# Z-T-WANG/DeepReinforcementLearningControlOfQuantumCartpoles

Hardware: AMD Instinct MI355X
Metric: env-steps/sec (whole node), inverted-harmonic grid=512 batch=65536; 1/2/4/8 GPU (higher is better)
Workload: dtype f64; 1 GPU; inverted_harmonic N=512 per-GPU batch=65536 dt=1/1440 80 physics steps + moments per step (metric); global_batch=65536, seq_len=512, parallelism=env-shard1, world_size_seen=1

## Files before the change

deepreinforcementlearningcontrolofquantumcartpoles_amd/csrc/qcart_api.cpp:

```cpp
#include <hip/hip_runtime.h>

#include <algorithm>
#include <cmath>
#include <cstdlib>
#include <cstring>
#include <mutex>
#include <string>
#include <vector>

#include "../../include/qcart.h"
#include "qcart_kargs.hpp"
#include "qcart_tables.hpp"

using namespace qcart;

namespace {
constexpr int kMaxSlots = 64;
constexpr int kShortCallSteps = 10;
constexpr int64_t kShortCallBatch = 4096;
constexpr int64_t kSpreadBatch = 1024;
std::mutex g_err_mu;
std::string g_create_err;

void set_create_err(const std::string& s) {
// ... 156 lines not shown
    if ((rc = upload(h, &h->d_kb, kb.data(), kb.size()))) return rc;
    return QC_OK;
}

int build_all_actions(qc_handle* h) {
    std::vector<double> forces;
    for (auto& a : h->acts) forces.push_back(a.force);
    if (forces.empty())
        for (int a = 0; a < h->p.n_actions; a++)
            forces.push_back((double)(a - h->p.n_actions / 2) * (h->p.f_max / (double)(h->p.n_actions / 2)));
    h->acts.assign(forces.size(), ActHost());
    for (size_t i = 0; i < forces.size(); i++) {
        int rc = build_action(h->op, h->p.dt, forces[i], h->mirror, h->acts[i], h->err);
        if (rc) return rc;
    }
    return QC_OK;
}

KArgs base_args(const qc_handle* h) {
    KArgs a;
    std::memset(&a, 0, sizeof(a));
    const qc_params& p = h->p;
    const OpHost& op = h->op;
    a.B = p.batch;
    a.env_offset = p.env_offset;
    a.seed = p.seed;
    a.ctr = h->d_ctr;
    a.N = op.N;
    a.Npad = op.Npad;
    a.n_slots = (int32_t)h->acts.size();
    a.mirror = h->mirror ? 1 : 0;
    a.bnd_len = op.fock ? kFockBnd : kGridBnd;
    a.win_lo = a.win_hi = 0;
    if (!op.fock && p.xth > 0) {
        const int c = op.N / 2, w = (int)std::nearbyint(p.xth / op.h);
        a.win_lo = c - w;
        a.win_hi = c + w;
    }
    a.moment_order = op.fock ? 0 : p.moment_order;
    {
        int lf = 0, lb = 0;
        for (auto& s : h->acts) {
            lf = std::max(lf, s.kf);
            lb = std::max(lb, s.kb);
        }
        const bool f32 = p.precision == QC_FP32;
        const uint32_t es = f32 ? 8u : 16u;
        const SlotLayout L = slot_layout(op.kl, op.Rs, op.family == QC_IHO, es, op.sym, op.lanes);
        const int NL = mode2_levels(op.kl);
        const size_t t1 = L.tf, t2 = L.tf + (size_t)(2 * NL + 2) * op.kl * op.kl * op.lanes * es;
        const size_t fx = op.fock ? (f32 ? 0 : (size_t)(op.R + 1 + (op.family == QC_IHO ? op.R : 0)) * kWave * 8)
                                  : (grid_rows_in_lds(op.R) ? (size_t)2 * op.R * kWave * 8 : 0);
        const size_t t4 = L.tf + (size_t)(NL + 1) * op.kl * op.kl * op.lanes * es;
        const size_t nzb = f32 ? 0 : (size_t)h->wpb * kNzLds, cap = 160 * 1024 - nzb;
        const bool m4 = !op.fock && !f32 && grid_rows_in_lds(op.R) && lf <= NL && t4 + fx <= cap;
        int mode = (t2 + fx <= cap && lf <= NL && lb <= NL) ? 2 : m4 ? 4 : (t1 + fx <= cap ? 1 : 0);
        if (const char* e = std::getenv("QCART_TAB_MODE")) {
            const int c = std::atoi(e);
            if (mode != 4 || c < 2) mode = std::min(mode, c);
        }
        a.tab_mode = mode;
        a.lds_fx = (uint32_t)(mode == 2 ? t2 : mode == 4 ? t4 : t1);
        a.lds_bytes = mode ? (uint32_t)(a.lds_fx + fx) : 0u;
        if (h->dual_img && mode >= 1) {
            a.lds_img = h->dual_img;
            a.lds_bytes = std::max(a.lds_bytes, 2u * h->dual_img);
        }
        a.lds_nz = 0;
        if (mode >= 1 && nzb) {
            a.lds_nz = (a.lds_bytes + 15u) & ~15u;
            a.lds_bytes = a.lds_nz + (uint32_t)nzb;
        }
    }
    a.precision = p.precision;
    a.order = nullptr;
    a.n_blocks = (uint32_t)((p.batch + h->wpb - 1) / h->wpb);
    a.n_obs = qc_n_obs(h);
    a.dt = p.dt;
    a.sqrt_dt = std::sqrt(p.dt);
    a.gamma = p.gamma;
    a.g4 = p.gamma / 4.;
    a.beta = std::sqrt(p.gamma / 2.);
    a.inv_sqrt2g = 1.0 / std::sqrt(2. * p.gamma);
    a.w = op.w;
    a.inv_sqrt_w = 1.0 / std::sqrt(op.w);
    a.c = op.c;
    a.h = op.fock ? 1.0 : op.h;
    const double dt = p.dt;
    a.x2h = op.family == QC_IHO ? -1.0 / op.c : 0.0;
    a.a2 = dt * dt * dt / 12.;
    a.a3 = dt * dt * dt * dt / 24.;
    a.a4 = dt * dt * dt * dt * dt / 80.;
    a.a5 = dt * dt * dt * dt * dt * dt / 360.;
    a.inv_sdt = 1.0 / a.sqrt_dt;
    a.inv_dt = 1.0 / dt;
    a.k_hisdt = 0.5 * a.inv_sdt;
    a.k_qisdt = 0.25 * a.inv_sdt;
    a.k_hidt = 0.5 * a.inv_dt;
    a.k_qidt = 0.25 * a.inv_dt;
    a.k_qdt = 0.25 * dt;
    a.k_qsdt = 0.25 * a.sqrt_dt;
    a.k_dz = a.sqrt_dt * dt * 0.5;
    a.k_sb = a.sqrt_dt * a.beta;
    a.b2 = a.a2 / a.a5;
    a.b3 = a.a3 / a.a5;
    a.b4 = a.a4 / a.a5;
    a.fail_thr = p.family == QC_HO ? 1e-3 : (p.family == QC_IHO ? 2e-3 : 5e-3);
// ... 699 lines not shown
```

deepreinforcementlearningcontrolofquantumcartpoles_amd/csrc/qcart_expt.hpp:

```cpp
#pragma once
#include <hip/hip_runtime.h>

#ifndef QCART_W8_MAX_R
#define QCART_W8_MAX_R 8
#endif
#ifndef QCART_W8_MAX_RG
#define QCART_W8_MAX_RG 9
#endif
#ifndef QCART_GRID_HC
#define QCART_GRID_HC 1
#endif
#ifndef QCART_GRID_KAR
#define QCART_GRID_KAR 0
#endif
#ifndef QCART_WKS_F32
#define QCART_WKS_F32 3
#endif
#ifndef QCART_SPLITM
#define QCART_SPLITM 1
#endif
#ifndef QCART_NZ_LDS
#define QCART_NZ_LDS 1
#endif
#ifndef QCART_MCONV_NT
#define QCART_MCONV_NT 2, 2, 1
#endif
#ifndef QCART_MCONV_NA
#define QCART_MCONV_NA 2, 1, 2
#endif
#ifndef QCART_MCONV_Q
#define QCART_MCONV_Q 4, 4, 4
#endif
#ifndef QCART_MFC_MT
#define QCART_MFC_MT 2
#endif
#ifndef QCART_MFC_NT
#define QCART_MFC_NT 2
#endif
#ifndef QCART_FC1_STAGE_K
#define QCART_FC1_STAGE_K 1
#endif

#ifdef QCART_STAMPS
namespace qcart {
__device__ unsigned long long qc_stamps[20];
}
#define QC_STAMP(ph)                                                                                 \
    do {                                                                                             \
        __builtin_amdgcn_sched_barrier(0);                                                           \
        unsigned long long t_;                                                                       \
        asm volatile("s_memtime %0\n\ts_waitcnt lgkmcnt(0)" : "=s"(t_)::"memory");                   \
        __builtin_amdgcn_sched_barrier(0);                                                           \
        st_acc[st_ph] += t_ - st_t;                                                                  \
        st_t = t_;                                                                                   \
        st_ph = (ph);                                                                                \
    } while (0)
#define QC_STAMP_BEGIN()                                                                             \
    unsigned long long st_acc[16] = {0}, st_t = 0;                                                   \
    int st_ph = 9;                                                                                   \
    asm volatile("s_memtime %0\n\ts_waitcnt lgkmcnt(0)" : "=s"(st_t)::"memory");                     \
    const unsigned long long st_loop0 = st_t
#define QC_KSTAMP_ENTRY()                                                                            \
    unsigned long long kst_t0;                                                                       \
    asm volatile("s_memtime %0\n\ts_waitcnt lgkmcnt(0)" : "=s"(kst_t0)::"memory")
#define QC_KSTAMP_EXIT(lane)                                                                         \
    do {                                                                                             \
        unsigned long long t_;                                                                       \
        asm volatile("s_memtime %0\n\ts_waitcnt lgkmcnt(0)" : "=s"(t_)::"memory");                   \
        if ((lane) == 0) {                                                                           \
            atomicAdd(&qc_stamps[16], st_loop0 - kst_t0);                                            \
            atomicAdd(&qc_stamps[17], t_ - st_t);                                                    \
            atomicAdd(&qc_stamps[18], 1ull);                                                         \
        }                                                                                            \
    } while (0)
#define QC_STAMP_END(lane)                                                                           \
// ... 47 lines not shown
```

deepreinforcementlearningcontrolofquantumcartpoles_amd/csrc/qcart_kargs.hpp:

```cpp
#pragma once
#include <stdint.h>

namespace qcart {

struct SlotLayout {
    uint32_t lc, uc, di, m2, tf, tb, bytes;
};
constexpr SlotLayout slot_layout(int kl, int R, bool has_m2, uint32_t es = 16, bool sym = false, int lanes = 64) {
    SlotLayout L{};
    const uint32_t ln = (uint32_t)lanes;
    L.lc = 0;
    L.uc = L.lc + es * ln * (uint32_t)(kl * R);
    L.di = L.uc + (sym ? 0u : es * ln * (uint32_t)(kl * R));
    L.m2 = L.di + es * ln * (uint32_t)R;
    L.tf = L.m2 + (has_m2 ? (es / 2) * ln * 10u * (uint32_t)R : 0u);
    L.tb = L.tf + es * ln * 7u * (uint32_t)(kl * kl);
    L.bytes = L.tb + es * ln * 7u * (uint32_t)(kl * kl);
    return L;
}

constexpr bool slot_sym(bool fock, uint32_t es, int lanes) { return !fock || lanes > 64 || es == 16; }

constexpr int mode2_levels(int kl) { return kl >= 4 ? 2 : 4; }
constexpr bool grid_rows_in_lds(int R) { return R >= 17; }
constexpr uint32_t kNzLds = 1024;

constexpr int kFockBnd = 5;
constexpr int kMaxMomentOrder = 9;
constexpr int kMaxMomentOrderHi = 16;
constexpr int kStepMaxMomentOrder = 6;
constexpr int kGridBnd = 6;

struct KArgs {
    void* psi;
    const int32_t* actions;
    const int32_t* env_steps;
    const double* noise;
    double* q_out;
    double* xm_out;
    int32_t* fail_step;
    int32_t* term_step;
    double* obs_out;
    int64_t B;
    int64_t env_offset;
    uint64_t seed;
    uint64_t* ctr;
    int32_t N;
    int32_t Npad;
    int32_t n_steps;
    int32_t default_action;
    int32_t n_slots;
    int32_t mirror;
    int32_t bnd_len;
    int32_t win_lo, win_hi;
    int32_t moment_order;
    int32_t n_obs;
    int32_t precision;
    int32_t tab_mode;
    uint32_t lds_bytes;
    uint32_t lds_fx;
    const int32_t* order;
    uint32_t n_blocks;
    const int32_t* order_mixed;
    uint32_t n_mixed;
    const int32_t* n_mixed_used;
    uint32_t lds_img;
    uint32_t lds_nz;
    double dt, sqrt_dt, gamma, g4, beta, inv_sqrt2g, w, inv_sqrt_w, c, h;
    double a2, a3, a4, a5;
    double fail_thr;
    double hoff[5];
    const double* xu;
    const double* xg;
    const double* hu;
    const double* tab;
    uint32_t slot_bytes;
    const int32_t* kf;
    const int32_t* kb;
// ... 100 lines not shown
```

deepreinforcementlearningcontrolofquantumcartpoles_amd/csrc/qcart_kernels.hpp:

```cpp
#pragma once
#include <hip/hip_runtime.h>
#include <stdint.h>

#include "qcart_expt.hpp"
#include "qcart_kargs.hpp"
#include "qcart_mt.hpp"
#include "qcart_shm.h"

namespace qcart {

template <typename RT>
struct cx {
    RT re, im;
};
typedef float v2f __attribute__((ext_vector_type(2)));
__device__ __forceinline__ v2f splat(float k) { return (v2f){k, k}; }
#ifdef QCART_F32_PACKED
constexpr bool kPackedF32 = true;
template <>
struct cx<float> {
    v2f v;
    __device__ __forceinline__ float get_re() const { return v.x; }
    __device__ __forceinline__ void put_re(float f) { v.x = f; }
    __device__ __forceinline__ float get_im() const { return v.y; }
// ... 1221 lines not shown
                char* fimg = img + (second ? a.lds_img : 0u) + lds_fx;
#pragma unroll
                for (int t = 0; t <= R; ++t) {
                    const int r = lane * R - 1 + t;
                    const double x = (r >= 0 && r < a.Npad) ? a.xu[r] : 0.0;
                    *(double*)(fimg + t * 512 + lane * 8) = -cFs * x;
                }
                if constexpr (FAM == 1) {
#pragma unroll
                    for (int t = 0; t < R; ++t) {
                        const int r = lane * R + t;
                        const double xl = (r >= 1 && r - 1 < a.Npad) ? a.xu[r - 1] : 0.0;
                        const double xr = r < a.Npad ? a.xu[r] : 0.0;
                        *(double*)(fimg + (R + 1 + t) * 512 + lane * 8) = xl * xl + xr * xr;
                    }
                }
            }
        }
        __syncthreads();
    }
    if (!active) return;
    auto steps_of = [&]() {
        int n = a.n_steps;
        if (MODE == 0) {
            n = budget0 < 0 ? 0 : (budget0 < n ? budget0 : n);
        } else if (a.env_steps) {
            const int e = a.env_steps[env];
            n = e < 0 ? 0 : (e < n ? e : n);
        }
        return __builtin_amdgcn_readfirstlane(n);
    };
    constexpr bool FROZEN_SKIP = SKIP && sizeof(RT) == 8;
    if (FROZEN_SKIP && !a.obs_out && !a.term_step && steps_of() == 0) {
        if (lane == 0 && a.fail_step) a.fail_step[env] = 0;
        return;
    }
    const int base = gl * R;
    const int lnv = lane;
    const int N = a.N;
    Coef<FAM, R, RT> cf;
    load_coef<FAM, R>(cf, a, base);

    RT* gpsi = (RT*)a.psi + (size_t)env * N * 2;
    if constexpr (!PRE && RES) {
        res_rows();
    } else if constexpr (!PRE) {
#pragma unroll
        for (int j = 0; j < R; ++j)
            psi[j] = (base + j < N) ? ld_cx<RT>(gpsi + 2 * (base + j)) : C(RT(0), RT(0));
    }

    const bool win_on = a.win_hi > a.win_lo;
    cx<RT> xp[FAM == 2 ? 1 : R];
    if constexpr (FAM != 2) apply_x<FAM, R>(psi, xp, cf, lnv);
    constexpr bool RCL = FAM == 2 && MODE >= 1 && grid_rows_in_lds(R);
    constexpr bool RGL = FAM == 2 && MODE == 0 && grid_rows_in_lds(R);
    RT hfd[FAM == 2 && !RCL && !RGL ? R : 1];
    if constexpr (FAM == 2 && !RCL && !RGL) {
#pragma unroll
        for (int j = 0; j < R; ++j) hfd[j] = cf.hu[j] - cF * cf.xg[j];
    }
    auto rowc = [&]() {
        if constexpr (RCL) {
            int vo = lane * 8;
            asm volatile("" : "+v"(vo));
            return RowLds<R>{(const char*)simg + a.lds_fx, vo};
        } else if constexpr (RGL) {
            int bo = base;
            asm volatile("" : "+v"(bo));
            return RowGlb<R>{a.hu, a.xg, cFd, bo};
        } else if constexpr (FAM == 2) {
            return RowReg<R>{hfd, cf.xg};
        } else {
            return 0;
        }
    };
    RT xbar;
    int term = -1, fail = 0;
    {
        double s[2] = {0.0, 0.0};
#pragma unroll
        for (int j = 0; j < R; ++j) {
            if constexpr (FAM == 2) s[0] += (double)(cf.xg[j] * (psi[j].re * psi[j].re + psi[j].im * psi[j].im));
            else s[0] += (double)(psi[j].re * xp[j].re + psi[j].im * xp[j].im);
            const int r = base + j;
            if (r >= a.win_lo && r < a.win_hi) s[1] += (double)(psi[j].re * psi[j].re + psi[j].im * psi[j].im);
        }
        step_sum<2>(s, lnv);
        xbar = (RT)(a.w * s[0]);
        if (win_on && 1.0 - s[1] * a.h > 0.5) term = 0;
    }
    constexpr bool HC = FAM != 2 || (QCART_GRID_HC && R < 17);
    const uint32_t genv = (uint32_t)(a.env_offset + env);
    constexpr bool NZL = MODE >= 1 && sizeof(RT) == 8 && QCART_NZ_LDS;
    double nz0 = 0.0, nz1 = 0.0;

    const int n_my = steps_of();
    const uint64_t ctr0 = a.ctr[env];
    constexpr bool KAR = !(FAM == 2 && R >= 17) || QCART_GRID_KAR;
    constexpr int SPD = (MODE >= 1 && (W == 4 || RES)) ? 4 : 0;
    const KArgs& a_in = a;
    constexpr bool LAZY = sizeof(RT) == 8;
    double scl = 1.0, sq = 1.0;
    QC_STAMP_BEGIN();
    for (int k = 0; k < n_my; ++k) {
        const auto& a = step_kargs<KAR>(a_in);
        const double dt = a.dt, sdt = a.sqrt_dt, g4 = a.g4, beta = a.beta;
        const double inv_sdt = HC ? a.inv_sdt : 1.0 / sdt, inv_dt = HC ? a.inv_dt : 1.0 / dt;
        const RT g4r = (RT)g4, dtr = (RT)dt, a5r = (RT)a.a5;
        const RT b2r = (RT)(HC ? a.b2 : a.a2 / a.a5), b3r = (RT)(HC ? a.b3 : a.a3 / a.a5),
                 b4r = (RT)(HC ? a.b4 : a.a4 / a.a5);
        QC_STAMP(0);
        if ((k & 63) == 0) {
            double z0 = 0.0, z1 = 0.0;
            if constexpr (RES) {
                z0 = lane == 0 ? rio->z0 : 0.0;
                z1 = lane == 0 ? rio->z1 : 0.0;
            } else if (a.noise) {
                const int kk = k + lane;
                if (kk < n_my) {
                    z0 = a.noise[((size_t)kk * a.B + env) * 2];
                    z1 = a.noise[((size_t)kk * a.B + env) * 2 + 1];
                }
            } else {
                normals(a.seed, genv, ctr0 + (uint64_t)(k + lane), 0u, z0, z1);
            }
            if constexpr (NZL) {
                *(double2*)(simg0 + a.lds_nz + ei * kNzLds + lane * 16) = make_double2(z0, z1);
                __builtin_amdgcn_fence(__ATOMIC_RELEASE, "wavefront");
                __builtin_amdgcn_wave_barrier();
            } else {
                nz0 = z0;
                nz1 = z1;
            }
        }
        double r0, r1;
        if constexpr (NZL) {
            const double2 z = *(const double2*)(simg0 + a.lds_nz + ei * kNzLds + (k & 63) * 16);
            r0 = readlane_d(z.x, 0);
            r1 = readlane_d(z.y, 0);
        } else {
            r0 = readlane_d(nz0, k & 63);
            r1 = readlane_d(nz1, k & 63);
        }
        const double dW = r0 * sdt, dZ = (HC ? a.k_dz : sdt * dt * 0.5) * (r0 + r1 * 0.57735026918962576451);
        if constexpr (RES) {
            rio->q = (double)xbar + dW * a.inv_sqrt2g * inv_dt;
            rio->xm = (double)xbar;
        } else if (lane == 0) {
            if (a.q_out) a.q_out[(size_t)k * a.B + env] = (double)xbar + dW * a.inv_sqrt2g * inv_dt;
            if (a.xm_out) a.xm_out[(size_t)k * a.B + env] = (double)xbar;
        }
        constexpr int EC = (int)sizeof(cx<RT>), ER = (int)sizeof(RT);
        int lane_o = gl, hc = gl * EC + 65536, hr = gl * ER + 65536, h2c = gl * EC + 131072, h2r = gl * ER + 131072;
        asm volatile("" : "+v"(lane_o), "+v"(hc), "+v"(hr));
        if constexpr (T2) asm volatile("" : "+v"(h2c), "+v"(h2r));
        const Tab<MODE, RT> tb{rs, (const char*)simg, lane_o * EC, lane_o * ER, hc, hr, h2c, h2r};
        double c1, c2, c3, c4, c5, c6;
        if constexpr (HC) {
            c1 = a.k_hisdt * dZ, c2 = a.k_qdt, c3 = a.k_qisdt * (dW * dW - dt);
            c4 = a.k_hidt * (dW * dt - dZ), c5 = a.k_qidt * (dW * dW * (1.0 / 3.0) - dt) * dW;
            c6 = a.k_qsdt * dW;
        } else {
            c1 = 0.5 * inv_sdt * dZ, c2 = 0.25 * dt, c3 = 0.25 * inv_sdt * (dW * dW - dt);
            c4 = 0.5 * inv_dt * (dW * dt - dZ), c5 = 0.25 * inv_dt * (dW * dW * (1.0 / 3.0) - dt) * dW;
            c6 = 0.25 * sdt * dW;
        }

        if constexpr (FAM == 2) {
            cx<RT> acc[R], D1[R];
            auto hf = [&](const cx<RT> (&v)[R], cx<RT> (&u)[R]) {
                const auto rc = rowc();
                grid_hf_rows<R>(v, rc, cf, lane, [&](int j, RT re, RT im) { u[j] = C(re, im); });
            };
            hf(psi, D1);
            {
            const auto rc = rowc();
#pragma unroll
            for (int j = 0; j < R; ++j) {
                const RT xr = (RT)rc.x(j) - xbar, q = g4r * xr * xr;
                D1[j] = C(D1[j].im - q * psi[j].re, -D1[j].re - q * psi[j].im);
            }
            }
            QC_STAMP(1);
            const RT kA = (RT)((dW - 2.0 * c4) * beta), k2 = (RT)(2.0 * c2), kY = (RT)(HC ? a.k_sb : sdt * beta);
            cx<RT> Ym[R];
            {
                cx<RT> t[R];
                hf(D1, acc);
#pragma unroll
                for (int j = 0; j < R; ++j) t[j] = C(-acc[j].im - b4r * D1[j].re, acc[j].re - b4r * D1[j].im);
                hf(t, acc);
#pragma unroll
                for (int j = 0; j < R; ++j) t[j] = C(acc[j].re + b3r * D1[j].im, acc[j].im - b3r * D1[j].re);
                hf(t, acc);
#pragma unroll
                for (int j = 0; j < R; ++j) t[j] = C(acc[j].re + b2r * D1[j].re, acc[j].im + b2r * D1[j].im);
                hf(t, acc);
                hf(acc, t);
                const auto rc = rowc();
#pragma unroll
                for (int j = 0; j < R; ++j) {
                    const RT xr = (RT)rc.x(j) - xbar;
                    const cx<RT> rl = C(xr * psi[j].re, xr * psi[j].im);
                    acc[j] = C(psi[j].re + kA * rl.re + k2 * D1[j].re + a5r * t[j].re,
                               psi[j].im + kA * rl.im + k2 * D1[j].im + a5r * t[j].im);
                    const cx<RT> y0 = C(psi[j].re + dtr * D1[j].re, psi[j].im + dtr * D1[j].im);
                    Ym[j] = C(y0.re - kY * rl.re, y0.im - kY * rl.im);
                    psi[j] = C(y0.re + kY * rl.re, y0.im + kY * rl.im);
                }
            }
            QC_STAMP(3);
            const RT kIm = (RT)(c1 - c6);
            const double kP = HC ? a.k_sb : sdt * beta;
            double yp, ym;
            {
                double sm[2] = {0.0, 0.0};
                const auto rc = rowc();
#pragma unroll
// ... 60 lines not shown
                const bool won = win_on && wh > wl;
                const int llo = wl / R, jlo = wl - llo * R, lhi = wh / R, jhi = wh - lhi * R;
                double s[3] = {0.0, 0.0, 0.0}, ct = 0.0, cl = 0.0, ch = 0.0, cb = 0.0;
                const auto rc = rowc();
#pragma unroll
                for (int j = R - 1; j >= 0; --j) {
                    const double p2 = (double)(acc[j].re * acc[j].re + acc[j].im * acc[j].im);
                    s[0] = j == R - 1 ? p2 : s[0] + p2;
                    s[1] += rc.x(j) * p2;
                    ct = fma(j == jt ? 1.0 : 0.0, s[0], ct);
                    cl = fma(j == jlo ? 1.0 : 0.0, s[0], cl);
                    ch = fma(j == jhi ? 1.0 : 0.0, s[0], ch);
                    if (j == JB) cb = s[0];
                }
                const double tot = s[0];
                if (won) {
                    const int l = lane;
                    double pw = (l > llo && l < lhi) ? tot : 0.0;
                    pw = l == llo ? (llo == lhi ? cl - ch : cl) : pw;
                    pw = (l == lhi && llo != lhi) ? tot - ch : pw;
                    s[2] = pw;
                }
                double stop = readlane_d(ct, lt), sbot = 0.0;
                for (int l = lt + 1; l <= (N - 1) / R; ++l) stop += readlane_d(tot, l);
#pragma unroll
                for (int l = 0; l < LB; ++l) sbot += readlane_d(tot, l);
                sbot += readlane_d(JB < R ? tot - cb : tot, LB);
                step_sum<3>(s);
                const double pwin = s[2];
                double scale = __builtin_amdgcn_rsq(s[0]);
                scale = scale * (1.5 - 0.5 * s[0] * scale * scale);
                scale = scale * (1.5 - 0.5 * s[0] * scale * scale);
                scale = scale * a.inv_sqrt_w;
#pragma unroll
                for (int j = 0; j < R; ++j) psi[j] = acc[j];
                scl = scale;
                sq = scale * scale;
                if (lazy_rescale(scl)) {
#pragma unroll
                    for (int j = 0; j < R; ++j) psi[j] = C(psi[j].re * (RT)scl, psi[j].im * (RT)scl);
                    scl = 1.0;
                    sq = 1.0;
                }
                xbar = (RT)(a.w * (s[1] * scale) * scale);
                const double sc2 = scale * scale, thr2 = a.fail_thr * a.fail_thr;
                const bool f = stop * sc2 > thr2 || sbot * sc2 > thr2;
                if (f && fail == 0) fail = k + 1;
                if (won && term < 0 && 1.0 - a.h * (pwin * scale) * scale > 0.5) term = k + 1;
            }
        } else {
        cx<RT> acc[R], rel[R], D1[R];
#pragma unroll
        for (int j = 0; j < R; ++j) rel[j] = C(xp[j].re - xbar * psi[j].re, xp[j].im - xbar * psi[j].im);
        apply_h<FAM, R>(psi, D1, cf, lnv);
#pragma unroll
        for (int j = 0; j < R; ++j)
            D1[j] = C(D1[j].im - cF * xp[j].im, -(D1[j].re - cF * xp[j].re));
        {
            cx<RT> xr[R];
            const RT gx = g4r * xbar;
            apply_x<FAM, R>(rel, xr, cf, lnv);
#pragma unroll
            for (int j = 0; j < R; ++j)
                D1[j] = C(D1[j].re - g4r * xr[j].re + gx * rel[j].re, D1[j].im - g4r * xr[j].im + gx * rel[j].im);
        }
        QC_STAMP(1);
        {
            auto hf = [&](const cx<RT> (&v)[R], cx<RT> (&u)[R]) {
                if constexpr (FXL) apply_hf_fx<FAM, R>(v, u, cf, tb, lds_fx, lnv);
                else apply_hf<FAM, R>(v, u, cF, cf, lnv);
            };
            cx<RT> t[R];
            hf(D1, acc);
#pragma unroll
            for (int j = 0; j < R; ++j) t[j] = C(-acc[j].im - b4r * D1[j].re, acc[j].re - b4r * D1[j].im);
            hf(t, acc);
#pragma unroll
            for (int j = 0; j < R; ++j) t[j] = C(acc[j].re + b3r * D1[j].im, acc[j].im - b3r * D1[j].re);
            hf(t, acc);
#pragma unroll
            for (int j = 0; j < R; ++j) t[j] = C(acc[j].re + b2r * D1[j].re, acc[j].im + b2r * D1[j].im);
            hf(t, acc);
            hf(acc, t);
            const RT kA = (RT)((dW - 2.0 * c4) * beta), k2 = (RT)(2.0 * c2);
#pragma unroll
            for (int j = 0; j < R; ++j) {
                acc[j] = C(psi[j].re + kA * rel[j].re + k2 * D1[j].re + a5r * t[j].re,
                           psi[j].im + kA * rel[j].im + k2 * D1[j].im + a5r * t[j].im);
                psi[j] = C(psi[j].re + dtr * D1[j].re, psi[j].im + dtr * D1[j].im);
            }
        }
        QC_STAMP(2);
        if constexpr (FAM == 1) {
            constexpr bool MPIPE = sizeof(RT) == 4 && R >= 32 && QCART_MPIPE;
            if (a.mirror && MPIPE) {
                constexpr int HB = QCART_MPIPE_ROWS, NB = 10 * R / HB, DP = QCART_MPIPE_DEPTH;
                static_assert(!MPIPE || (R % HB == 0 && DP >= 2), "mirror batches: whole fractions of a band");
                cx<RT> lo[10];
                make_lo<R, 10>(D1, lo, lnv);
                RT mb[DP][HB];
                auto rd = [&](int q, RT (&dst)[HB]) {
#pragma unroll
                    for (int i = 0; i < HB; ++i)
                        dst[i] = tb.d(SL.m2 + (uint32_t)((q * HB / R) * R + (q * HB) % R + i) * CR);
                };
#pragma unroll
                for (int q = 0; q < DP - 1; ++q) rd(q, mb[q]);
#pragma unroll
                for (int q = 0; q < NB; ++q) {
                    if (q + DP - 1 < NB) rd(q + DP - 1, mb[(q + DP - 1) % DP]);
                    __builtin_amdgcn_sched_barrier(0);
                    const int d = q * HB / R + 1;
#pragma unroll
                    for (int i = 0; i < HB; ++i) {
                        const int j = (q * HB) % R + i;
                        const RT m = mb[q % DP][i];
                        const cx<RT> dv = (j - d >= 0) ? D1[(j - d) >= 0 ? (j - d) : 0]
                                                   : lo[(10 + j - d) < 10 ? (10 + j - d) : 0];
                        acc[j] = C(acc[j].re + m * dv.im, acc[j].im - m * dv.re);
                    }
                }
            } else if (a.mirror) {
                constexpr int MB = 1;
                cx<RT> lo[10];
                make_lo<R, 10>(D1, lo, lnv);
#pragma unroll
                for (int h = 0; h < 10 / MB; ++h) {
                    RT mv[MB][R];
#pragma unroll
                    for (int dd = 0; dd < MB; ++dd)
#pragma unroll
                        for (int j = 0; j < R; ++j) mv[dd][j] = tb.d(SL.m2 + (uint32_t)((MB * h + dd) * R + j) * CR);
                    __builtin_amdgcn_sched_barrier(0);
#pragma unroll
                    for (int j = 0; j < R; ++j)
#pragma unroll
                        for (int dd = 0; dd < MB; ++dd) {
                            const int d = MB * h + dd + 1;
                            const cx<RT> dv = (j - d >= 0) ? D1[(j - d) >= 0 ? (j - d) : 0]
                                                       : lo[(10 + j - d) < 10 ? (10 + j - d) : 0];
                            acc[j] = C(acc[j].re + mv[dd][j] * dv.im, acc[j].im - mv[dd][j] * dv.re);
                        }
                }
            }
        }
        QC_STAMP(3);
        const RT kY = (RT)(HC ? a.k_sb : sdt * beta), kIm = (RT)(c1 - c6);
        const double kP = HC ? a.k_sb : sdt * beta;
        constexpr bool X2H = FAM == 1 && ((FXL && R <= 8) || sizeof(RT) == 4);
        auto xdiag = [&](int j) -> RT {
            if constexpr (FXL) return *(const RT*)(tb.lds + tb.vr + lds_fx + (R + 1 + j) * 64 * (int)sizeof(RT));
            else return cf.xu[j] * cf.xu[j] + cf.xu[j + 1] * cf.xu[j + 1];
        };
        constexpr bool SPLITM = sizeof(RT) == 4 && R >= 32 && QCART_SPLITM;
        cx<RT> xYp[R];
        double yp = 0.0, ym, s1p = 0.0;
        {
            cx<RT> Ym[R], xYm[R];
#pragma unroll
            for (int j = 0; j < R; ++j) {
                Ym[j] = C(psi[j].re - kY * rel[j].re, psi[j].im - kY * rel[j].im);
                psi[j] = C(psi[j].re + kY * rel[j].re, psi[j].im + kY * rel[j].im);
            }
            apply_x<FAM, R>(Ym, xYm, cf, lnv);
            if constexpr (SPLITM) {
                RowDot<RT> q1;
#pragma unroll
                for (int j = 0; j < R; ++j) q1.add(j == 0, Ym[j], xYm[j]);
                double sm[1] = {q1.sum()};
                step_sum<1>(sm, lnv);
                ym = (a.w * sq) * sm[0];
            } else {
                apply_x<FAM, R>(psi, xYp, cf, lnv);
                RowDot<RT> q0, q1;
#pragma unroll
                for (int j = 0; j < R; ++j) {
                    q0.add(j == 0, psi[j], xYp[j]);
                    q1.add(j == 0, Ym[j], xYm[j]);
                }
                double sm[2] = {q0.sum(), q1.sum()};
                step_sum<2>(sm, lnv);
                yp = (a.w * sq) * sm[0];
                ym = (a.w * sq) * sm[1];
                s1p = sm[0];
            }
            const RT ymr = (RT)ym;
            if constexpr (X2H) {
                const double kRed = -(c2 - c1) * g4, kDmd = (c4 - c3 + c5) * beta - kRed * ym;
                const RT kRe = (RT)kRed, kH = (RT)(kRed * a.x2h), kX = (RT)(kDmd - kRed * ym), nk = (RT)(-kDmd * ym),
                         kIc = kIm * cF;
                h_rows<FAM, R>(Ym, cf, lnv, [&](int j, RT hre, RT him) {
                    const RT cy = kRe * xdiag(j) + nk;
                    acc[j] = C(acc[j].re + kH * hre - kIm * him + cy * Ym[j].re + kX * xYm[j].re + kIc * xYm[j].im,
                               acc[j].im + kH * him + kIm * hre + cy * Ym[j].im + kX * xYm[j].im - kIc * xYm[j].re);
                });
            } else {
            {
                h_rows<FAM, R>(Ym, cf, lnv, [&](int j, RT hre, RT him) {
                    hre -= cF * xYm[j].re;
                    him -= cF * xYm[j].im;
                    acc[j] = C(acc[j].re - kIm * him, acc[j].im + kIm * hre);
                    xYm[j] = C(xYm[j].re - ymr * Ym[j].re, xYm[j].im - ymr * Ym[j].im);
                });
            }
            apply_x<FAM, R>(xYm, Ym, cf, lnv);
            const double kRed = -(c2 - c1) * g4;
            const RT kRe = (RT)kRed, kDm = (RT)((c4 - c3 + c5) * beta - kRed * ym);
#pragma unroll
            for (int j = 0; j < R; ++j)
                acc[j] = C(acc[j].re + kRe * Ym[j].re + kDm * xYm[j].re, acc[j].im + kRe * Ym[j].im + kDm * xYm[j].im);
            }
        }
        if constexpr (SPLITM) {
            apply_x<FAM, R>(psi, xYp, cf, lnv);
            RowDot<RT> q0;
#pragma unroll
            for (int j = 0; j < R; ++j) q0.add(j == 0, psi[j], xYp[j]);
            double sm[1] = {q0.sum()};
            step_sum<1>(sm, lnv);
            yp = (a.w * sq) * sm[0];
            s1p = sm[0];
        }
        QC_STAMP(4);
        if constexpr (X2H) {
            cx<RT> t[R];
            const RT al = (RT)a.x2h, kIc = kIm * cF;
            RowDot<RT> q2, q3;
            h_rows<FAM, R>(psi, cf, lnv, [&](int j, RT hre, RT him) {
                acc[j] = C(acc[j].re + kIm * him - kIc * xYp[j].im, acc[j].im - kIm * hre + kIc * xYp[j].re);
                const RT dj = xdiag(j);
                t[j] = C(al * hre + dj * psi[j].re, al * him + dj * psi[j].im);
                q2.add(j == 0, xYp[j], xYp[j]);
                q3.add(j == 0, xYp[j], t[j]);
            });
            double d2[2] = {q2.sum(), q3.sum()};
            step_sum<2>(d2, lnv);
            QC_STAMP(6);
            const double kRed = -(c1 + c2) * g4, kDpd = (c3 + c4 - c5) * beta - kRed * yp, k5 = c5 * beta;
            const double wq = a.w * sq;
            const double p0 = 2.0 * (d2[0] - yp * s1p), p1 = d2[1] - 2.0 * yp * d2[0] + yp * yp * s1p;
            const double dpm = 2.0 * wq * kP * p0, spm = 2.0 * yp + 2.0 * wq * kP * kP * p1;
            const double fxd = kRed + 2.0 * k5 * kP, frd = kDpd - k5 * kP * spm, fyd = -k5 * dpm;
            const RT fx = (RT)fxd, fy = (RT)(fyd - frd * yp), fr = (RT)(frd - fxd * yp);
#pragma unroll
            for (int j = 0; j < R; ++j)
                acc[j] = C(acc[j].re + fx * t[j].re + fy * psi[j].re + fr * xYp[j].re,
                           acc[j].im + fx * t[j].im + fy * psi[j].im + fr * xYp[j].im);
        } else {
            cx<RT> rp[R], xrp[R];
            const RT ypr = (RT)yp;
            h_rows<FAM, R>(psi, cf, lnv, [&](int j, RT hre, RT him) {
                hre -= cF * xYp[j].re;
                him -= cF * xYp[j].im;
                acc[j] = C(acc[j].re + kIm * him, acc[j].im - kIm * hre);
                rp[j] = C(xYp[j].re - ypr * psi[j].re, xYp[j].im - ypr * psi[j].im);
            });
            apply_x<FAM, R>(rp, xrp, cf, lnv);
            const double kRed = -(c1 + c2) * g4, kDpd = (c3 + c4 - c5) * beta - kRed * yp;
            QC_STAMP(5);
            RowDot<RT> q0, q1;
#pragma unroll
            for (int j = 0; j < R; ++j) {
                q0.add(j == 0, psi[j], xrp[j]);
                q0.add(false, rp[j], xYp[j]);
                q1.add(j == 0, rp[j], xrp[j]);
            }
            double d2[2] = {q0.sum(), q1.sum()};
            step_sum<2>(d2, lnv);
            QC_STAMP(6);
            const double k5 = c5 * beta;
            const double wq = a.w * sq;
            const double dpm = 2.0 * wq * kP * d2[0], spm = 2.0 * yp + 2.0 * wq * kP * kP * d2[1];
            const RT fx = (RT)(kRed + 2.0 * k5 * kP), fy = (RT)(-k5 * dpm), fr = (RT)(kDpd - k5 * kP * spm);
#pragma unroll
            for (int j = 0; j < R; ++j)
                acc[j] = C(acc[j].re + fx * xrp[j].re + fy * psi[j].re + fr * rp[j].re,
                           acc[j].im + fx * xrp[j].im + fy * psi[j].im + fr * rp[j].im);
        }
        QC_STAMP(7);
        band_solve<KL, R, MODE, FAM == 1, SYMT, LE, SPD>(acc, tb, kf, kb, lnv QC_SOLVE_STAMP_PASS);
        QC_STAMP(8);
        {
            cx<RT> xn[R];
            apply_x<FAM, R>(acc, xn, cf, lnv);
            double s[2] = {0.0, 0.0}, pwin = 0.0, stop = 0.0, sbot = 0.0;
            if constexpr (FAM <= 1) {
                const int r0 = N - a.bnd_len, lt = r0 / R, jt = r0 - lt * R;
                double suf = 0.0;
                RowDot<RT> qx;
#pragma unroll
                for (int j = R - 1; j >= 0; --j) {
                    s[0] = dot_acc(s[0], j == R - 1, acc[j], acc[j]);
                    qx.add(j == R - 1, acc[j], xn[j]);
                    suf = fma(j == jt ? 1.0 : 0.0, s[0], suf);
                }
                s[1] = qx.sum();
                const int l1 = (N - 1) / R;
                if (lt < 64) stop = readlane_d(suf, lt);
                for (int l = lt + 1; l <= l1 && l < 64; ++l) stop += readlane_d(s[0], l);
            } else {
                double ptop = 0.0, pbot = 0.0;
#pragma unroll
                for (int j = 0; j < R; ++j) {
                    const double p2 = (double)(acc[j].re * acc[j].re + acc[j].im * acc[j].im);
                    s[0] += p2;
                    s[1] += (double)(acc[j].re * xn[j].re + acc[j].im * xn[j].im);
                    const int r = base + j;
                    if (r >= N - a.bnd_len && r < N) ptop += p2;
                    if (r < a.bnd_len) pbot += p2;
                    if (r >= a.win_lo && r < a.win_hi) pwin += p2;
                }
                for (int l = (N - a.bnd_len) / R; l <= (N - 1) / R; ++l) stop += readlane_d(ptop, l);
                for (int l = 0; l <= (a.bnd_len - 1) / R; ++l) sbot += readlane_d(pbot, l);
            }
            step_sum<2>(s);
            double scale = __builtin_amdgcn_rsq(s[0]);
            scale = scale * (1.5 - 0.5 * s[0] * scale * scale);
            scale = scale * (1.5 - 0.5 * s[0] * scale * scale);
            if constexpr (FAM == 2) scale = scale * a.inv_sqrt_w;
#pragma unroll
            for (int j = 0; j < R; ++j) {
                psi[j] = LAZY ? acc[j] : C(acc[j].re * (RT)scale, acc[j].im * (RT)scale);
                xp[j] = LAZY ? xn[j] : C(xn[j].re * (RT)scale, xn[j].im * (RT)scale);
            }
            if constexpr (LAZY) {
                scl = scale;
                sq = scale * scale;
                if (lazy_rescale(scl)) {
#pragma unroll
                    for (int j = 0; j < R; ++j) {
                        psi[j] = C(psi[j].re * (RT)scl, psi[j].im * (RT)scl);
                        xp[j] = C(xp[j].re * (RT)scl, xp[j].im * (RT)scl);
                    }
                    scl = 1.0;
                    sq = 1.0;
                }
            }
            xbar = (RT)(a.w * (s[1] * scale) * scale);
            const double sc2 = scale * scale, thr2 = a.fail_thr * a.fail_thr;
            bool f = stop * sc2 > thr2;
            if constexpr (FAM == 2) f = f || (sbot * sc2 > thr2);
            if (f && fail == 0) fail = k + 1;
            if constexpr (FAM == 2) {
                if (win_on && term < 0) {
                    double sw[1] = {pwin};
                    step_sum<1>(sw);
                    if (1.0 - a.h * (sw[0] * scale) * scale > 0.5) term = k + 1;
                }
            }
        }
        }
    }
    QC_STAMP_END(lane);
    if constexpr (LAZY) {
#pragma unroll
        for (int j = 0; j < R; ++j) psi[j] = C(psi[j].re * (RT)scl, psi[j].im * (RT)scl);
    }
    if (!FROZEN_SKIP || n_my > 0) {
        int wb = gl * R;
        asm volatile("" : "+v"(wb));
#pragma unroll
        for (int j = 0; j < R; ++j)
            if (wb + j < N) st_cx<RT>(gpsi + 2 * (wb + j), psi[j]);
        if constexpr (RES) {
            cx<RT>* rl = (cx<RT>*)((char*)smem_dyn + rio->lds_row);
#pragma unroll
            for (int j = 0; j < R; ++j) rl[j * 64 + lane] = psi[j];
        }
    }
    if constexpr (RES) {
        rio->fail = fail;
    } else if (lane == 0) {
        if (a.fail_step) a.fail_step[env] = fail;
        if (a.term_step) a.term_step[env] = term;
        if (!a.noise) a.ctr[env] = ctr0 + (uint64_t)n_my;
    }
    if (a.obs_out) {
        if constexpr (FAM <= 1) {
            double o[5];
            fock_obs<FAM, R>(psi, cf, lnv, o);
            if (lane < 5) {
                double v = o[0];
#pragma unroll
                for (int i = 1; i < 5; ++i) v = (lane == i) ? o[i] : v;
                a.obs_out[(size_t)env * 5 + lane] = v;
            }
// ... 482 lines not shown
    } else if (kind == 1) {
        const int levels = (int)a0;
        double s[1] = {0.0};
#pragma unroll
        for (int j = 0; j < R; ++j) {
            const int r = base + j;
            if (r < levels && r < N) {
                double r0, r1;
                normals(a.seed, (uint32_t)(a.env_offset + env), (uint64_t)r, 1u, r0, r1);
                v[j] = C(r0, r1);
                s[0] += r0 * r0 + r1 * r1;
            } else {
                v[j] = C(0.0, 0.0);
            }
        }
        wave_sum<1>(s);
        const double sc = 1.0 / sqrt(s[0]);
#pragma unroll
        for (int j = 0; j < R; ++j) v[j] = C(v[j].re * sc, v[j].im * sc);
    } else {
        const double k = k_arr ? k_arr[env] : a0, mu = m_arr ? m_arr[env] : a1, sg = s_arr ? s_arr[env] : a2;
        const double nrm = sqrt(sqrt(2.0 * M_PI) * sg);
#pragma unroll
        for (int j = 0; j < R; ++j) {
            const int r = base + j;
            const double x = (r < N) ? a.xg[r] : 0.0;
            const double ph = 2.0 * M_PI * (x - mu) * k;
            const double g = exp(-(x - mu) * (x - mu) / (4.0 * sg * sg)) / nrm;
            double sn, cs;
            sincos(ph, &sn, &cs);
            v[j] = C(cs * g, sn * g);
        }
    }
#pragma unroll
    for (int j = 0; j < R; ++j)
        if (base + j < N) {
            gpsi[2 * (base + j)] = (RT)v[j].re;
            gpsi[2 * (base + j) + 1] = (RT)v[j].im;
        }
}

}

namespace qcart {

static inline unsigned nblocks(int64_t B) { return (unsigned)((B + 3) / 4); }

template <int FAM, int R, typename RT>
constexpr uint32_t kDualImg =
    slot_layout(Fam<FAM>::KL, R, FAM == 1, (uint32_t)sizeof(cx<RT>), slot_sym(FAM != 2, (uint32_t)sizeof(cx<RT>), 64), 64).tf +
    (FAM <= 1 ? (uint32_t)(R + 1 + (FAM == 1 ? R : 0)) * 64u * 8u : 0u);
template <int FAM, int R, typename RT>
constexpr bool kDual = sizeof(RT) == 8 && !(FAM == 2 && grid_rows_in_lds(R)) &&
                      2u * ((kDualImg<FAM, R, RT> + 15u) & ~15u) + (uint32_t)kStepWaves<FAM, R, RT> * kNzLds <= 160u * 1024u;

template <int FAM, int R>
constexpr bool kMode4 = FAM == 2 && grid_rows_in_lds(R);

template <int FAM, int R, int MODE, typename RT, bool DUAL = false>
int launch_step_mode(const KArgs& a, hipStream_t st) {
    const dim3 grid(a.n_blocks + (DUAL ? a.n_mixed : 0u)), block(64 * kStepWaves<FAM, R, RT>);
    constexpr bool lds = MODE >= 1;
    if (lds) {
        static bool attr_set = false;
        if (!attr_set) {
            if (hipFuncSetAttribute((const void*)k_step<FAM, R, MODE, RT, DUAL>,
                                    hipFuncAttributeMaxDynamicSharedMemorySize, 160 * 1024) != hipSuccess)
                return -3;
            attr_set = true;
        }
    }
    hipLaunchKernelGGL((k_step<FAM, R, MODE, RT, DUAL>), grid, block, lds ? a.lds_bytes : 0, st, a);
    return 0;
}
template <int FAM, int R, typename RT = double>
int launch_one(int kind, const KArgs& a, int what, double xth, void* out, int rkind, const uint8_t* mask,
               double a0, double a1, double a2, const double* k_arr, const double* m_arr, const double* s_arr,
               void* stream) {
    const dim3 grid(nblocks(a.B)), block(256);
    hipStream_t st = (hipStream_t)stream;
    if (kind == 4) return kStepWaves<FAM, R, RT>;
    if (kind == 8) return (kResident<FAM, R> && sizeof(RT) == 8) ? 1 : 0;
    if (kind == 7) {
        if constexpr (kResident<FAM, R> && sizeof(RT) == 8) {
            if (a.tab_mode == 2) {
                if constexpr (FAM <= 1) {
                    static bool attr_set = false;
                    if (!attr_set) {
                        if (hipFuncSetAttribute((const void*)k_resident<FAM, R, 2>,
                                                hipFuncAttributeMaxDynamicSharedMemorySize,
                                                156 * 1024) != hipSuccess)
                            return -3;
                        attr_set = true;
                    }
                    hipLaunchKernelGGL((k_resident<FAM, R, 2>), dim3((unsigned)a.B), dim3(64), a.lds_bytes, st, a,
                                       *(const ResArgs*)out);
                } else {
                    return -6;
                }
            } else {
                hipLaunchKernelGGL((k_resident<FAM, R, 0>), dim3((unsigned)a.B), dim3(64), a.lds_bytes, st, a,
                                   *(const ResArgs*)out);
            }
            return hipGetLastError() == hipSuccess ? 0 : -3;
        }
        return -6;
    }
// ... 53 lines not shown
```

Measured before the change: 224.1 million env-steps/s.

## Precompute per-step noise coefficients in LDS and fuse H/x stencils in IHO step

```diff
diff --git a/deepreinforcementlearningcontrolofquantumcartpoles_amd/csrc/qcart_api.cpp b/deepreinforcementlearningcontrolofquantumcartpoles_amd/csrc/qcart_api.cpp
--- a/deepreinforcementlearningcontrolofquantumcartpoles_amd/csrc/qcart_api.cpp
+++ b/deepreinforcementlearningcontrolofquantumcartpoles_amd/csrc/qcart_api.cpp
@@ -232,7 +232,7 @@
         const size_t fx = op.fock ? (f32 ? 0 : (size_t)(op.R + 1 + (op.family == QC_IHO ? op.R : 0)) * kWave * 8)
                                   : (grid_rows_in_lds(op.R) ? (size_t)2 * op.R * kWave * 8 : 0);
         const size_t t4 = L.tf + (size_t)(NL + 1) * op.kl * op.kl * op.lanes * es;
-        const size_t nzb = f32 ? 0 : (size_t)h->wpb * kNzLds, cap = 160 * 1024 - nzb;
+        const size_t nzb = f32 ? 0 : (size_t)h->wpb * nz_lds(op.fock), cap = 160 * 1024 - nzb;
         const bool m4 = !op.fock && !f32 && grid_rows_in_lds(op.R) && lf <= NL && t4 + fx <= cap;
         int mode = (t2 + fx <= cap && lf <= NL && lb <= NL) ? 2 : m4 ? 4 : (t1 + fx <= cap ? 1 : 0);
         if (const char* e = std::getenv("QCART_TAB_MODE")) {
diff --git a/deepreinforcementlearningcontrolofquantumcartpoles_amd/csrc/qcart_expt.hpp b/deepreinforcementlearningcontrolofquantumcartpoles_amd/csrc/qcart_expt.hpp
--- a/deepreinforcementlearningcontrolofquantumcartpoles_amd/csrc/qcart_expt.hpp
+++ b/deepreinforcementlearningcontrolofquantumcartpoles_amd/csrc/qcart_expt.hpp
@@ -21,6 +21,12 @@
 #endif
 #ifndef QCART_NZ_LDS
 #define QCART_NZ_LDS 1
+#endif
+#ifndef QCART_NZ_COEF
+#define QCART_NZ_COEF 1
+#endif
+#ifndef QCART_ROT
+#define QCART_ROT 1
 #endif
 #ifndef QCART_MCONV_NT
 #define QCART_MCONV_NT 2, 2, 1
diff --git a/deepreinforcementlearningcontrolofquantumcartpoles_amd/csrc/qcart_kargs.hpp b/deepreinforcementlearningcontrolofquantumcartpoles_amd/csrc/qcart_kargs.hpp
--- a/deepreinforcementlearningcontrolofquantumcartpoles_amd/csrc/qcart_kargs.hpp
+++ b/deepreinforcementlearningcontrolofquantumcartpoles_amd/csrc/qcart_kargs.hpp
@@ -24,6 +24,8 @@
 constexpr int mode2_levels(int kl) { return kl >= 4 ? 2 : 4; }
 constexpr bool grid_rows_in_lds(int R) { return R >= 17; }
 constexpr uint32_t kNzLds = 1024;
+constexpr uint32_t kNzSteps = 32, kNzFock = 7;
+constexpr uint32_t nz_lds(bool fock) { return fock ? kNzSteps * kNzFock * 8u : kNzLds; }
 
 constexpr int kFockBnd = 5;
 constexpr int kMaxMomentOrder = 9;
diff --git a/deepreinforcementlearningcontrolofquantumcartpoles_amd/csrc/qcart_kernels.hpp b/deepreinforcementlearningcontrolofquantumcartpoles_amd/csrc/qcart_kernels.hpp
--- a/deepreinforcementlearningcontrolofquantumcartpoles_amd/csrc/qcart_kernels.hpp
+++ b/deepreinforcementlearningcontrolofquantumcartpoles_amd/csrc/qcart_kernels.hpp
@@ -1297,7 +1297,10 @@
 
     const bool win_on = a.win_hi > a.win_lo;
     cx<RT> xp[FAM == 2 ? 1 : R];
-    if constexpr (FAM != 2) apply_x<FAM, R>(psi, xp, cf, lnv);
+    constexpr bool ROT = FAM == 1 && sizeof(RT) == 8 && !RES && QCART_ROT && W == 8;
+    cx<RT> hp[ROT ? R : 1];
+    if constexpr (ROT) apply_hx<FAM, R>(psi, hp, xp, cf, lnv);
+    else if constexpr (FAM != 2) apply_x<FAM, R>(psi, xp, cf, lnv);
     constexpr bool RCL = FAM == 2 && MODE >= 1 && grid_rows_in_lds(R);
     constexpr bool RGL = FAM == 2 && MODE == 0 && grid_rows_in_lds(R);
     RT hfd[FAM == 2 && !RCL && !RGL ? R : 1];
@@ -1338,6 +1341,12 @@
     constexpr bool HC = FAM != 2 || (QCART_GRID_HC && R < 17);
     const uint32_t genv = (uint32_t)(a.env_offset + env);
     constexpr bool NZL = MODE >= 1 && sizeof(RT) == 8 && QCART_NZ_LDS;
+    constexpr bool NZK = NZL && FAM <= 1 && !RES && QCART_NZ_COEF && MODE != 1 && W == 8;
+    constexpr int NZP = NZK ? (int)kNzSteps : 64;
+    constexpr uint32_t NZB = NZK ? nz_lds(true) : kNzLds;
+    constexpr uint32_t NZ_KC = 0, NZ_TK = 16 * kNzSteps, NZ_KA = 32 * kNzSteps, NZ_TM = 40 * kNzSteps,
+                       NZ_QD = 48 * kNzSteps;
+    static_assert(!NZK || NZ_QD + 8 * kNzSteps == nz_lds(true), "the parked coefficients fill the wave's buffer");
     double nz0 = 0.0, nz1 = 0.0;
 
     const int n_my = steps_of();
@@ -1356,7 +1365,25 @@
         const RT b2r = (RT)(HC ? a.b2 : a.a2 / a.a5), b3r = (RT)(HC ? a.b3 : a.a3 / a.a5),
                  b4r = (RT)(HC ? a.b4 : a.a4 / a.a5);
         QC_STAMP(0);
-        if ((k & 63) == 0) {
+        auto wiener = [&](const auto& ka, double r0, double r1, double& dW, double& dZ) {
+            dW = r0 * sdt, dZ = (HC ? ka.k_dz : sdt * dt * 0.5) * (r0 + r1 * 0.57735026918962576451);
+        };
+        auto noise_coefs = [&](const auto& ka, double dW, double dZ, double& c1, double& c2, double& c3, double& c4,
+                               double& c5, double& c6) {
+            if constexpr (HC) {
+                c1 = ka.k_hisdt * dZ, c2 = ka.k_qdt, c3 = ka.k_qisdt * (dW * dW - dt);
+                c4 = ka.k_hidt * (dW * dt - dZ), c5 = ka.k_qidt * (dW * dW * (1.0 / 3.0) - dt) * dW;
+                c6 = ka.k_qsdt * dW;
+            } else {
+                c1 = 0.5 * inv_sdt * dZ, c2 = 0.25 * dt, c3 = 0.25 * inv_sdt * (dW * dW - dt);
+                c4 = 0.5 * inv_dt * (dW * dt - dZ), c5 = 0.25 * inv_dt * (dW * dW * (1.0 / 3.0) - dt) * dW;
+                c6 = 0.25 * sdt * dW;
+            }
+        };
+        auto nzw = [&]() { return simg0 + a.lds_nz + ei * NZB; };
+        auto nzk1 = [&, k](uint32_t off) { return *(const double*)(nzw() + off + (k & (NZP - 1)) * 8); };
+        auto nzk2 = [&, k](uint32_t off) { return *(const double2*)(nzw() + off + (k & (NZP - 1)) * 16); };
+        if ((k & (NZP - 1)) == 0) {
             double z0 = 0.0, z1 = 0.0;
             if constexpr (RES) {
                 z0 = lane == 0 ? rio->z0 : 0.0;
@@ -1368,10 +1395,29 @@
                     z1 = a.noise[((size_t)kk * a.B + env) * 2 + 1];
                 }
             } else {
-                normals(a.seed, genv, ctr0 + (uint64_t)(k + lane), 0u, z0, z1);
-            }
-            if constexpr (NZL) {
-                *(double2*)(simg0 + a.lds_nz + ei * kNzLds + lane * 16) = make_double2(z0, z1);
+                uint32_t ge = genv;
+                if constexpr (NZK) asm volatile("" : "+s"(ge));
+                normals(a.seed, ge, ctr0 + (uint64_t)(k + lane), 0u, z0, z1);
+            }
+            if constexpr (NZK) {
+                const KArgs* av = (const KArgs*)__builtin_amdgcn_kernarg_segment_ptr();
+                asm volatile("" : "+v"(av));
+                double dW, dZ, c1, c2, c3, c4, c5, c6;
+                wiener(*av, z0, z1, dW, dZ);
+                noise_coefs(*av, dW, dZ, c1, c2, c3, c4, c5, c6);
+                const double kAd = (dW - 2.0 * c4) * beta, kImd = c1 - c6, tm = c4 - c3 + c5, tp = c3 + c4 - c5,
+                             k5 = c5 * beta, qd = dW * av->inv_sqrt2g;
+                if (lane < NZP) {
+                    *(double2*)(nzw() + NZ_KC + lane * 16) = make_double2(kImd, c1);
+                    *(double2*)(nzw() + NZ_TK + lane * 16) = make_double2(tp, k5);
+                    *(double*)(nzw() + NZ_KA + lane * 8) = kAd;
+                    *(double*)(nzw() + NZ_TM + lane * 8) = tm;
+                    *(double*)(nzw() + NZ_QD + lane * 8) = qd;
+                }
+                __builtin_amdgcn_fence(__ATOMIC_RELEASE, "wavefront");
+                __builtin_amdgcn_wave_barrier();
+            } else if constexpr (NZL) {
+                *(double2*)(nzw() + lane * 16) = make_double2(z0, z1);
                 __builtin_amdgcn_fence(__ATOMIC_RELEASE, "wavefront");
                 __builtin_amdgcn_wave_barrier();
             } else {
@@ -1379,21 +1425,28 @@
                 nz1 = z1;
             }
         }
-        double r0, r1;
-        if constexpr (NZL) {
-            const double2 z = *(const double2*)(simg0 + a.lds_nz + ei * kNzLds + (k & 63) * 16);
-            r0 = readlane_d(z.x, 0);
-            r1 = readlane_d(z.y, 0);
-        } else {
-            r0 = readlane_d(nz0, k & 63);
-            r1 = readlane_d(nz1, k & 63);
-        }
-        const double dW = r0 * sdt, dZ = (HC ? a.k_dz : sdt * dt * 0.5) * (r0 + r1 * 0.57735026918962576451);
+        double dW = 0.0, dZ = 0.0;
+        if constexpr (!NZK) {
+            double r0, r1;
+            if constexpr (NZL) {
+                const double2 z = *(const double2*)(nzw() + (k & 63) * 16);
+                r0 = readlane_d(z.x, 0);
+                r1 = readlane_d(z.y, 0);
+            } else {
+                r0 = readlane_d(nz0, k & 63);
+                r1 = readlane_d(nz1, k & 63);
+            }
+            wiener(a, r0, r1, dW, dZ);
+        }
         if constexpr (RES) {
             rio->q = (double)xbar + dW * a.inv_sqrt2g * inv_dt;
             rio->xm = (double)xbar;
         } else if (lane == 0) {
-            if (a.q_out) a.q_out[(size_t)k * a.B + env] = (double)xbar + dW * a.inv_sqrt2g * inv_dt;
+            if constexpr (NZK) {
+                if (a.q_out) a.q_out[(size_t)k * a.B + env] = (double)xbar + nzk1(NZ_QD) * inv_dt;
+            } else {
+                if (a.q_out) a.q_out[(size_t)k * a.B + env] = (double)xbar + dW * a.inv_sqrt2g * inv_dt;
+            }
             if (a.xm_out) a.xm_out[(size_t)k * a.B + env] = (double)xbar;
         }
         constexpr int EC = (int)sizeof(cx<RT>), ER = (int)sizeof(RT);
@@ -1401,15 +1454,12 @@
         asm volatile("" : "+v"(lane_o), "+v"(hc), "+v"(hr));
         if constexpr (T2) asm volatile("" : "+v"(h2c), "+v"(h2r));
         const Tab<MODE, RT> tb{rs, (const char*)simg, lane_o * EC, lane_o * ER, hc, hr, h2c, h2r};
-        double c1, c2, c3, c4, c5, c6;
-        if constexpr (HC) {
-            c1 = a.k_hisdt * dZ, c2 = a.k_qdt, c3 = a.k_qisdt * (dW * dW - dt);
-            c4 = a.k_hidt * (dW * dt - dZ), c5 = a.k_qidt * (dW * dW * (1.0 / 3.0) - dt) * dW;
-            c6 = a.k_qsdt * dW;
+        double c1 = 0.0, c2 = 0.0, c3 = 0.0, c4 = 0.0, c5 = 0.0, c6 = 0.0;
+        if constexpr (NZK) {
+            static_assert(!NZK || HC, "the parked coefficients are the host-folded forms'");
+            c2 = a.k_qdt;
         } else {
-            c1 = 0.5 * inv_sdt * dZ, c2 = 0.25 * dt, c3 = 0.25 * inv_sdt * (dW * dW - dt);
-            c4 = 0.5 * inv_dt * (dW * dt - dZ), c5 = 0.25 * inv_dt * (dW * dW * (1.0 / 3.0) - dt) * dW;
-            c6 = 0.25 * sdt * dW;
+            noise_coefs(a, dW, dZ, c1, c2, c3, c4, c5, c6);
         }
 
         if constexpr (FAM == 2) {
@@ -1576,7 +1626,12 @@
         cx<RT> acc[R], rel[R], D1[R];
 #pragma unroll
         for (int j = 0; j < R; ++j) rel[j] = C(xp[j].re - xbar * psi[j].re, xp[j].im - xbar * psi[j].im);
-        apply_h<FAM, R>(psi, D1, cf, lnv);
+        if constexpr (ROT) {
+#pragma unroll
+            for (int j = 0; j < R; ++j) D1[j] = hp[j];
+        } else {
+            apply_h<FAM, R>(psi, D1, cf, lnv);
+        }
 #pragma unroll
         for (int j = 0; j < R; ++j)
             D1[j] = C(D1[j].im - cF * xp[j].im, -(D1[j].re - cF * xp[j].re));
@@ -1606,7 +1661,10 @@
             for (int j = 0; j < R; ++j) t[j] = C(acc[j].re + b2r * D1[j].re, acc[j].im + b2r * D1[j].im);
             hf(t, acc);
             hf(acc, t);
-            const RT kA = (RT)((dW - 2.0 * c4) * beta), k2 = (RT)(2.0 * c2);
+            RT kA;
+            if constexpr (NZK) kA = (RT)nzk1(NZ_KA);
+            else kA = (RT)((dW - 2.0 * c4) * beta);
+            const RT k2 = (RT)(2.0 * c2);
 #pragma unroll
             for (int j = 0; j < R; ++j) {
                 acc[j] = C(psi[j].re + kA * rel[j].re + k2 * D1[j].re + a5r * t[j].re,
@@ -1669,7 +1727,15 @@
             }
         }
         QC_STAMP(3);
-        const RT kY = (RT)(HC ? a.k_sb : sdt * beta), kIm = (RT)(c1 - c6);
+        const RT kY = (RT)(HC ? a.k_sb : sdt * beta);
+        RT kIm;
+        if constexpr (NZK) {
+            const double2 kc = nzk2(NZ_KC);
+            kIm = (RT)kc.x;
+            c1 = kc.y;
+        } else {
+            kIm = (RT)(c1 - c6);
+        }
         const double kP = HC ? a.k_sb : sdt * beta;
         constexpr bool X2H = FAM == 1 && ((FXL && R <= 8) || sizeof(RT) == 4);
         auto xdiag = [&](int j) -> RT {
@@ -1710,7 +1776,8 @@
             }
             const RT ymr = (RT)ym;
             if constexpr (X2H) {
-                const double kRed = -(c2 - c1) * g4, kDmd = (c4 - c3 + c5) * beta - kRed * ym;
+                const double kRed = -(c2 - c1) * g4, tm = NZK ? nzk1(NZ_TM) : c4 - c3 + c5;
+                const double kDmd = tm * beta - kRed * ym;
                 const RT kRe = (RT)kRed, kH = (RT)(kRed * a.x2h), kX = (RT)(kDmd - kRed * ym), nk = (RT)(-kDmd * ym),
                          kIc = kIm * cF;
                 h_rows<FAM, R>(Ym, cf, lnv, [&](int j, RT hre, RT him) {
@@ -1729,7 +1796,9 @@
             }
             apply_x<FAM, R>(xYm, Ym, cf, lnv);
             const double kRed = -(c2 - c1) * g4;
-            const RT kRe = (RT)kRed, kDm = (RT)((c4 - c3 + c5) * beta - kRed * ym);
+            const RT kRe = (RT)kRed;
+            const double tm = NZK ? nzk1(NZ_TM) : c4 - c3 + c5;
+            const RT kDm = (RT)(tm * beta - kRed * ym);
 #pragma unroll
             for (int j = 0; j < R; ++j)
                 acc[j] = C(acc[j].re + kRe * Ym[j].re + kDm * xYm[j].re, acc[j].im + kRe * Ym[j].im + kDm * xYm[j].im);
@@ -1760,7 +1829,14 @@
             double d2[2] = {q2.sum(), q3.sum()};
             step_sum<2>(d2, lnv);
             QC_STAMP(6);
-            const double kRed = -(c1 + c2) * g4, kDpd = (c3 + c4 - c5) * beta - kRed * yp, k5 = c5 * beta;
+            double tp = 0.0, k5p = 0.0;
+            if constexpr (NZK) {
+                const double2 tk = nzk2(NZ_TK);
+                tp = tk.x, k5p = tk.y;
+            }
+            const double kRed = -(c1 + c2) * g4;
+            if constexpr (!NZK) tp = c3 + c4 - c5;
+            const double kDpd = tp * beta - kRed * yp, k5 = NZK ? k5p : c5 * beta;
             const double wq = a.w * sq;
             const double p0 = 2.0 * (d2[0] - yp * s1p), p1 = d2[1] - 2.0 * yp * d2[0] + yp * yp * s1p;
             const double dpm = 2.0 * wq * kP * p0, spm = 2.0 * yp + 2.0 * wq * kP * kP * p1;
@@ -1780,7 +1856,14 @@
                 rp[j] = C(xYp[j].re - ypr * psi[j].re, xYp[j].im - ypr * psi[j].im);
             });
             apply_x<FAM, R>(rp, xrp, cf, lnv);
-            const double kRed = -(c1 + c2) * g4, kDpd = (c3 + c4 - c5) * beta - kRed * yp;
+            double tp = 0.0, k5p = 0.0;
+            if constexpr (NZK) {
+                const double2 tk = nzk2(NZ_TK);
+                tp = tk.x, k5p = tk.y;
+            }
+            const double kRed = -(c1 + c2) * g4;
+            if constexpr (!NZK) tp = c3 + c4 - c5;
+            const double kDpd = tp * beta - kRed * yp;
             QC_STAMP(5);
             RowDot<RT> q0, q1;
 #pragma unroll
@@ -1792,7 +1875,7 @@
             double d2[2] = {q0.sum(), q1.sum()};
             step_sum<2>(d2, lnv);
             QC_STAMP(6);
-            const double k5 = c5 * beta;
+            const double k5 = NZK ? k5p : c5 * beta;
             const double wq = a.w * sq;
             const double dpm = 2.0 * wq * kP * d2[0], spm = 2.0 * yp + 2.0 * wq * kP * kP * d2[1];
             const RT fx = (RT)(kRed + 2.0 * k5 * kP), fy = (RT)(-k5 * dpm), fr = (RT)(kDpd - k5 * kP * spm);
@@ -1805,8 +1888,16 @@
         band_solve<KL, R, MODE, FAM == 1, SYMT, LE, SPD>(acc, tb, kf, kb, lnv QC_SOLVE_STAMP_PASS);
         QC_STAMP(8);
         {
-            cx<RT> xn[R];
-            apply_x<FAM, R>(acc, xn, cf, lnv);
+            cx<RT> xn[R], hn[ROT ? R : 1], eh[ROT ? R + 4 : 1];
+            if constexpr (ROT) {
+                make_ext<R, 2>(acc, eh, lnv);
+#pragma unroll
+                for (int j = 0; j < R; ++j)
+                    xn[j] = C(cf.xu[j + 1] * eh[j + 3].re + cf.xu[j] * eh[j + 1].re,
+                              cf.xu[j + 1] * eh[j + 3].im + cf.xu[j] * eh[j + 1].im);
+            } else {
+                apply_x<FAM, R>(acc, xn, cf, lnv);
+            }
             double s[2] = {0.0, 0.0}, pwin = 0.0, stop = 0.0, sbot = 0.0;
             if constexpr (FAM <= 1) {
                 const int r0 = N - a.bnd_len, lt = r0 / R, jt = r0 - lt * R;
@@ -1838,6 +1929,12 @@
                 for (int l = 0; l <= (a.bnd_len - 1) / R; ++l) sbot += readlane_d(pbot, l);
             }
             step_sum<2>(s);
+            if constexpr (ROT) {
+#pragma unroll
+                for (int j = 0; j < R; ++j)
+                    hn[j] = C(cf.hu[j + 2] * eh[j + 4].re + cf.hu[j] * eh[j].re,
+                              cf.hu[j + 2] * eh[j + 4].im + cf.hu[j] * eh[j].im);
+            }
             double scale = __builtin_amdgcn_rsq(s[0]);
             scale = scale * (1.5 - 0.5 * s[0] * scale * scale);
             scale = scale * (1.5 - 0.5 * s[0] * scale * scale);
@@ -1846,6 +1943,7 @@
             for (int j = 0; j < R; ++j) {
                 psi[j] = LAZY ? acc[j] : C(acc[j].re * (RT)scale, acc[j].im * (RT)scale);
                 xp[j] = LAZY ? xn[j] : C(xn[j].re * (RT)scale, xn[j].im * (RT)scale);
+                if constexpr (ROT) hp[j] = hn[j];
             }
             if constexpr (LAZY) {
                 scl = scale;
@@ -1856,6 +1954,7 @@
                         psi[j] = C(psi[j].re * (RT)scl, psi[j].im * (RT)scl);
                         xp[j] = C(xp[j].re * (RT)scl, xp[j].im * (RT)scl);
                     }
+                    if constexpr (ROT) apply_h<FAM, R>(psi, hp, cf, lnv);
                     scl = 1.0;
                     sq = 1.0;
                 }
@@ -2444,7 +2543,7 @@
     (FAM <= 1 ? (uint32_t)(R + 1 + (FAM == 1 ? R : 0)) * 64u * 8u : 0u);
 template <int FAM, int R, typename RT>
 constexpr bool kDual = sizeof(RT) == 8 && !(FAM == 2 && grid_rows_in_lds(R)) &&
-                      2u * ((kDualImg<FAM, R, RT> + 15u) & ~15u) + (uint32_t)kStepWaves<FAM, R, RT> * kNzLds <= 160u * 1024u;
+                      2u * ((kDualImg<FAM, R, RT> + 15u) & ~15u) + (uint32_t)kStepWaves<FAM, R, RT> * nz_lds(FAM <= 1) <= 160u * 1024u;
 
 template <int FAM, int R>
 constexpr bool kMode4 = FAM == 2 && grid_rows_in_lds(R);
```

Result: no change. 226.0 million env-steps/s (median of 6 runs) (+0.8%).
